# IVRL/NoiseDiff

Measured on AMD Instinct MI355X. Metric: sampled RAW patches/sec (256x256x4, 1000-step DDPM), higher is better.
Workload: dtype f32; 1 GPU; NoiseDiffNet dim=64, 256x256x4 patches, 1000-step DDPM (sigmoid2, pred_v), 16 patches per GPU; a step = one reverse-diffusion step (U-Net forward + fused posterior/noise update) over the per-GPU batch; patches/s = n_gpus*16/(1000*s_per_step); global_batch=16, launch=hipGraph replay, noise=device Philox4x32-10

## Files before the change

noisediff_amd/csrc/conv3x3_wino4.hip:

```cpp
#include <stdlib.h>
#include <type_traits>
#include "nd_common.h"

namespace {

typedef float f32x2 __attribute__((ext_vector_type(2)));
typedef unsigned u32x4_t __attribute__((ext_vector_type(4)));
typedef __attribute__((address_space(3))) void* lds_ptr;
typedef __attribute__((address_space(3))) short* lds_short_ptr;
typedef __attribute__((address_space(3))) unsigned* lds_u32_ptr;
typedef __attribute__((address_space(3))) unsigned short* lds_u16_ptr;
typedef __attribute__((address_space(3))) f32x4* lds_f32x4_ptr;

constexpr int KC4 = 16;
constexpr int NPOS = 36;
constexpr int VD_FLOATS = NPOS * 256;

constexpr int MAX_COUT = 2048;
template <int NTG, int NW = 4>
struct W4Geo {
    static constexpr int NT = 64 * NW;
    static constexpr int TGW = NTG * 4 / NW;
    static constexpr int REG_W = 16 * NTG, HALO_W = REG_W + 2;
    static constexpr int RAW_ROWP = NTG == 2 ? 40 : 24;
// ... 22 lines not shown
#ifndef W4_UR_GEN
#define W4_UR_GEN 6
#endif
#ifndef W4_UR_EPI
#define W4_UR_EPI 6
#endif
#ifndef W4_VR
#define W4_VR 3
#endif
#ifndef W4_COMMIT_AT
#define W4_COMMIT_AT 8
#endif
#ifndef W4_XF_AT
#define W4_XF_AT 10
#endif
#ifndef W4_U_AUX
#define W4_U_AUX 0
#endif
#ifndef W4_STORE_AUX
#define W4_STORE_AUX 19
#endif
#ifndef W4_STAGGER
#define W4_STAGGER 12
#endif
#ifndef W4_XF_SPLIT
#define W4_XF_SPLIT 1
#endif
#ifndef W4_UR1
#define W4_UR1 9
#endif
#ifndef W4_UR1_AFF
#define W4_UR1_AFF 6
#endif
#ifndef W4_UR1_EPI
#define W4_UR1_EPI 0
#endif
#ifndef W4_UR1_XF
#define W4_UR1_XF 6
#endif
#ifndef W4_PAIR_SKEW
#define W4_PAIR_SKEW 2
#endif
#ifndef W4_PRIO
#define W4_PRIO 0
#endif
#ifndef W4_ABLATE
#define W4_ABLATE 0
#endif

struct Wino4Args {
    nd_conv3x3 d;
    int tiles_x, tiles_y, regions_x, n_tiles, n_cg, n_c8, slots, total_wg;
    int splits, chunks_per_split;
};

#ifndef W4_NOP
#define W4_NOP ""
#endif
#define W4_MFMA_A(acc, uv, vv)  asm volatile(W4_NOP "v_mfma_f32_16x16x4_f32 %0, %2, %1, %0" : "+a"(acc) : "v"(uv), "v"(vv))
#define W4_MFMA_V(acc, uv, vv)  asm volatile(W4_NOP "v_mfma_f32_16x16x4_f32 %0, %2, %1, %0" : "+v"(acc) : "v"(uv), "v"(vv))
#define W4_MFMA_AZ(acc, uv, vv) asm volatile(W4_NOP "v_mfma_f32_16x16x4_f32 %0, %2, %1, 0" : "=&a"(acc) : "v"(uv), "v"(vv))
#define W4_MFMA_VZ(acc, uv, vv) asm volatile(W4_NOP "v_mfma_f32_16x16x4_f32 %0, %2, %1, 0" : "=&v"(acc) : "v"(uv), "v"(vv))
#define W4_MFMA_DRAIN() asm volatile("s_nop 15\n\ts_nop 15" ::: "memory")

__device__ __forceinline__ void w4_bt(const f32x2 (&d)[6], f32x2 (&t)[6]) {
    const f32x2 c4 = {4.0f, 4.0f}, cm4 = {-4.0f, -4.0f}, cm5 = {-5.0f, -5.0f}, c2 = {2.0f, 2.0f}, cm2 = {-2.0f, -2.0f};
    const f32x2 p = __builtin_elementwise_fma(cm4, d[2], d[4]), q = __builtin_elementwise_fma(cm4, d[1], d[3]);
    const f32x2 r = d[4] - d[2], s = d[3] - d[1];
    t[0] = __builtin_elementwise_fma(c4, d[0], __builtin_elementwise_fma(cm5, d[2], d[4]));
    t[1] = p + q;
    t[2] = p - q;
    t[3] = __builtin_elementwise_fma(c2, s, r);
    t[4] = __builtin_elementwise_fma(cm2, s, r);
    t[5] = __builtin_elementwise_fma(c4, d[1], __builtin_elementwise_fma(cm5, d[3], d[5]));
}

template <int HALF>
__device__ __forceinline__ void w4_bt_half(const f32x2 (&d)[6], f32x2 (&t)[3]) {
    const f32x2 c4 = {4.0f, 4.0f}, cm4 = {-4.0f, -4.0f}, cm5 = {-5.0f, -5.0f}, c2 = {2.0f, 2.0f}, cm2 = {-2.0f, -2.0f};
    if (HALF == 0) {
        const f32x2 p = __builtin_elementwise_fma(cm4, d[2], d[4]), q = __builtin_elementwise_fma(cm4, d[1], d[3]);
        t[0] = __builtin_elementwise_fma(c4, d[0], __builtin_elementwise_fma(cm5, d[2], d[4]));
        t[1] = p + q;
        t[2] = p - q;
    } else {
        const f32x2 r = d[4] - d[2], s = d[3] - d[1];
        t[0] = __builtin_elementwise_fma(c2, s, r);
        t[1] = __builtin_elementwise_fma(cm2, s, r);
        t[2] = __builtin_elementwise_fma(c4, d[1], __builtin_elementwise_fma(cm5, d[3], d[5]));
    }
}

template <int MODE, bool STREAM, bool SPLIT = false, int NTG = 2, int NW = 4>
__global__ __launch_bounds__((64 * NW), (W4Geo<NTG, NW>::WG_PER_CU)) void wino4_kernel(const Wino4Args a) {
    using Geo = W4Geo<NTG, NW>;
    constexpr int NT = Geo::NT, TGW = Geo::TGW;
    constexpr int RAW_FLOATS = Geo::RAW_FLOATS, BIAS_OFF_BYTES = Geo::BIAS_OFF_BYTES, ACC_AGPR = Geo::ACC_AGPR, REG_W = Geo::REG_W, HALO_W = Geo::HALO_W;
    constexpr bool MAP = MODE == ND_PRO_AFFINE_MAP_SILU;
    constexpr bool GEN = MODE == ND_PRO_AFFINE_GENMAP_SILU;
    constexpr bool MAPX = MAP || GEN;
    constexpr bool AFF = MODE == ND_PRO_AFFINE_SILU || MAPX;
    constexpr bool LEAKY = MODE == ND_PRO_LEAKY || MODE == ND_PRO_LEAKY_SECOND;
    constexpr int UR = TGW == 1 ? (AFF ? W4_UR1_AFF : W4_UR1) : MAP ? W4_UR_MAP : GEN ? W4_UR_GEN : AFF ? W4_UR_AFF : W4_UR, UR_EPI = TGW == 1 ? W4_UR1_EPI : W4_UR_EPI;
    static_assert(TGW == 2 || !MAPX, "the map prologues (20 more staging registers per halo item in flight) stay on the 512-register form");
    extern __shared__ __attribute__((aligned(16))) float lds_[];
    float* const Vd = lds_ + RAW_FLOATS;

    const int tid = threadIdx.x, lane = tid & 63;
    const int wave = __builtin_amdgcn_readfirstlane(tid >> 6);
    const int mtg = NW == 8 ? wave >> 2 : 0;
    const int tg = TGW == 2 ? wave >> 1 : mtg, rh = (wave >> 1) & 1, ch2 = wave & 1;
    const int tile = lane & 15, kq = lane >> 4;

    const int wgid = nd_xcd_remap(blockIdx.x, gridDim.x);
    const int t_begin = (int)((long)wgid * a.total_wg / gridDim.x), t_end = (int)((long)(wgid + 1) * a.total_wg / gridDim.x);
    if (t_begin >= t_end) return;

#ifdef W4_STAMP
    const unsigned long long stamp_c0 = __builtin_amdgcn_s_memtime(), stamp_r0 = __builtin_amdgcn_s_memrealtime();
    unsigned long long stamp_epi = 0, stamp_xf = 0, stamp_wait = 0, stamp_t = 0, stamp_drain = 0, stamp_first = 0, stamp_last = 0, stamp_second = 0, stamp_third = 0, stamp_pro = 0, stamp_top = 0, stamp_tile = 0;
#define W4_T0() (stamp_t = __builtin_amdgcn_s_memtime())
#define W4_ACC(x) (x += __builtin_amdgcn_s_memtime() - stamp_t)
#else
#define W4_T0()
#define W4_ACC(x)
#endif
#if W4_STAGGER
    if (a.total_wg >= 4 * (int)gridDim.x)
        for (int k = (int)(blockIdx.x >> 3) & 15; k > 0; --k) __builtin_amdgcn_s_sleep(W4_STAGGER);
#endif
#if W4_PAIR_SKEW
    if (NTG == 1 && 2 * blockIdx.x >= gridDim.x)
        for (int k = 0; k < W4_PAIR_SKEW; ++k) __builtin_amdgcn_s_sleep(32);
#endif
    const nd_src& s = a.d.src;
    const int H = a.d.H, W = a.d.W, Cin = a.d.cin, Cout = a.d.cout;
    const int up = s.upsample ? 1 : 0;
    const int sH = H >> up, sW = W >> up;
    const int Ctot = s.c0 + s.c1;
    const int n_chunks = SPLIT ? a.chunks_per_split : (Cin + KC4 - 1) / KC4;

    auto decode = [&](int t, int& b_, int& ty_, int& rx_, int& nt_, int& sp_) {
        int lid = t;
        nt_ = lid % a.n_tiles;  lid /= a.n_tiles;
        rx_ = lid % a.regions_x;  lid /= a.regions_x;
        ty_ = lid % a.tiles_y;
        b_ = lid / a.tiles_y;
        sp_ = 0;
        if (SPLIT) { sp_ = b_ / a.d.B;  b_ -= sp_ * a.d.B; }
    };

    constexpr int RAW_ROWP = Geo::RAW_ROWP, RAW_IT = Geo::RAW_IT;
    const long npx = (long)a.d.B * sH * sW;
    const unsigned PX_MARK = (unsigned)(npx + sW + 2);
    auto src_rsrc = [&](const float* p, long px_stride_floats) {
        return __builtin_amdgcn_make_buffer_rsrc(const_cast<float*>(p) - (long)(sW + 1) * px_stride_floats, 0,
                                                 (int)((npx + sW + 1) * px_stride_floats * 4), 0x00020000);
    };
    const __amdgpu_buffer_rsrc_t rsrc0 = src_rsrc(s.p0, s.ld0);
    const __amdgpu_buffer_rsrc_t rsrc1 = s.p1 ? src_rsrc(s.p1, s.ld1) : rsrc0;
    const __amdgpu_buffer_rsrc_t rsrcm = MAP ? src_rsrc(s.map, 2 * Ctot) : GEN ? src_rsrc(s.map, 8) : rsrc0;
    const int map_shift = s.map_blocked ? 64 : Ctot * 4;
    float* const vd_tg = Vd + tg * VD_FLOATS;
    char* const rawbuf = reinterpret_cast<char*>(lds_);
    lds_u32_ptr const ptab = (lds_u32_ptr)(Vd + NTG * VD_FLOATS) + tid;
    auto cperm = [](int c) { return ((c >> 2) & 3) | ((c & 3) << 2) | (c & 48); };
    auto swz = [](int r, int c) { return (2 * ((r >> 2) & 3)) ^ (4 * ((c >> 3) & 1)); };
    auto pixl_of = [](int t) { return GEN ? 16 * (t >> 6) + (t & 15) : t >> 2; };
    const int sq = GEN ? (tid >> 4) & 3 : tid & 3;
    lds_u32_ptr const rtab = ptab + RAW_IT * NT;
    lds_u16_ptr const dtab = (lds_u16_ptr)(ptab - tid + (Geo::RTAB ? 2 : 1) * RAW_IT * NT) + tid;
    lds_u16_ptr const ttab = dtab + RAW_IT * NT;
    float* const bias_lds = reinterpret_cast<float*>(reinterpret_cast<char*>(lds_) + BIAS_OFF_BYTES);
    auto item_rc = [&](int k, int tid_) {
        const int pix = pixl_of(tid_) + (NT / 4) * k, r = pix / HALO_W, c = pix - HALO_W * r;
        const int dy = up ? (r + 1) >> 1 : r, dx = up ? (c + 1) >> 1 : c;
        return (unsigned)(dy * sW + dx) | ((unsigned)r << 16) | ((unsigned)c << 24);
    };
#pragma unroll
    for (int k = 0; k < RAW_IT; ++k) {
        const int pix = pixl_of(tid) + (NT / 4) * k, r = pix / HALO_W, c = pix - HALO_W * r;
        dtab[k * NT] = (unsigned short)((r * RAW_ROWP + cperm(c)) * 64 + (((2 * sq) ^ swz(r, c)) * 8));
        if (Geo::RTAB) rtab[k * NT] = item_rc(k, tid);
    }
    const int t_tile = ((lane >> 1) & 7) | ((lane >> 4) & 1) << 3, t_kq = (lane & 1) | ((lane >> 5) << 1);
#pragma unroll
    for (int h = 0; h < 2; ++h)
#pragma unroll
        for (int bx = 0; bx < 6; ++bx) {
            const int r0 = 4 * (t_tile >> 2) + 4 * h, c = 16 * tg + 4 * (t_tile & 3) + bx;
            ttab[(h * 6 + bx) * NT] = (unsigned short)((4 * (t_tile >> 2) * RAW_ROWP + cperm(c)) * 64 + (((4 * ch2 + t_kq) ^ swz(r0, c)) * 8));
        }
    const unsigned t_lds = (unsigned)(ch2 * 1024 + (t_kq >> 1) * 512 + t_tile * 32 + (t_kq & 1) * 16);
    if (Geo::BIAS_LDS)
        for (int i = tid; i < a.n_tiles * 64; i += NT) bias_lds[i] = (a.d.bias && i < Cout) ? a.d.bias[i] : 0.0f;
    const __amdgpu_buffer_rsrc_t brsrc = __builtin_amdgcn_make_buffer_rsrc(const_cast<float*>(a.d.bias ? a.d.bias : a.d.weight), 0, a.d.bias ? Cout * 4 : 0, 0x00020000);
    float bias_r = 0.0f;

    const unsigned OOB = 0x7FFFFFF0u;
    int sb_ = 0;
    unsigned spx_ = 0;
    bool tab_clean = false;
    f32x4 tA4 = {1, 1, 1, 1}, tD4 = {0, 0, 0, 0};
    auto stage_tile = [&](int b_, int ty_, int rx_) {
        sb_ = b_;
        spx_ = (unsigned)((b_ * sH + ((ty_ * 16) >> up)) * sW + ((rx_ * REG_W) >> up));
        const int r_lo = ty_ == 0 ? 1 : 0, r_n = min(17, H - ty_ * 16) - r_lo;
        const int c_lo = rx_ == 0 ? 1 : 0, c_n = min(HALO_W - 1, W - rx_ * REG_W) - c_lo;
        const bool interior = r_lo == 0 && r_n == 17 && c_lo == 0 && c_n == HALO_W - 1;
        if (!(interior && tab_clean)) {
            int tid_ = tid;
            if (!Geo::RTAB) asm volatile("" : "+v"(tid_));
#pragma unroll
            for (int k = 0; k < RAW_IT; ++k) {
                const unsigned rc = Geo::RTAB ? rtab[k * NT] : item_rc(k, tid_);
                const unsigned r = (rc >> 16) & 255u, c = rc >> 24;
                const bool ok = r - (unsigned)r_lo <= (unsigned)r_n && c - (unsigned)c_lo <= (unsigned)c_n;
                ptab[k * NT] = ok ? (rc & 0xFFFFu) : PX_MARK;
            }
        }
        tab_clean = interior;
    };
    f32x4 raw[RAW_IT];
    constexpr int GEN_H = RAW_IT / 2;
    f32x4 msc[MAP ? RAW_IT : GEN ? GEN_H : 1], msh[MAP ? RAW_IT : GEN ? GEN_H : 1];
    float ev0[GEN ? RAW_IT : 1], ev1[GEN ? RAW_IT : 1];
    float gw_sc0 = 0, gw_sc1 = 0, gw_sh0 = 0, gw_sh1 = 0;
    f32x4 gb_sc = {0, 0, 0, 0}, gb_sh = {0, 0, 0, 0};
    int i_eoff = 0;
    bool i_second = false;
    __amdgpu_buffer_rsrc_t i_rs = rsrc0;
    int i_soff = 0, i_mapoff = 0;
    unsigned i_ld4 = 0, i_bias = 0;
    auto stage_issue_begin = [&](int cb_) {
        const bool sec = cb_ >= s.c0;
        i_second = sec;
        i_mapoff = (int)(cb_ * (s.map_blocked ? 8u : 4u) + spx_ * (unsigned)(2 * Ctot * 4));
        i_rs = sec ? rsrc1 : rsrc0;
        i_ld4 = (unsigned)(sec ? s.ld1 : s.ld0) * 4u;
        i_soff = (int)((sec ? cb_ - s.c0 : cb_) * 4u + spx_ * i_ld4);
        i_bias = cb_ + 4 * sq < Cin ? 16u * sq : OOB;
        if (GEN) {
            i_eoff = (int)(spx_ * 32u);
            const float* wr = s.gamma + (size_t)(cb_ + (lane & 15)) * 8 + sq;
            gw_sc0 = wr[0];  gw_sc1 = wr[4];  gw_sh0 = wr[(size_t)Ctot * 8];  gw_sh1 = wr[(size_t)Ctot * 8 + 4];
            gb_sc = nd_ld4(s.beta + cb_ + 4 * sq);  gb_sh = nd_ld4(s.beta + Ctot + cb_ + 4 * sq);
        }
        if (AFF) {
            const int c = cb_ + 4 * sq;
            const float* m = s.mad + (size_t)sb_ * 3 * Ctot + (c < Cin ? c : 0);
            const f32x4 M = nd_ld4(m), A = nd_ld4(m + Ctot), D = nd_ld4(m + 2 * Ctot);
            tA4 = A;
            tD4 = D - M * A;
        }
    };
    auto stage_issue_one = [&](int k, unsigned px, auto tile_first_c) {
#if !(W4_ABLATE & 1)
        const unsigned voff = __umul24(px, i_ld4) + i_bias;
        raw[k] = __builtin_bit_cast(f32x4, __builtin_amdgcn_raw_buffer_load_b128(i_rs, voff, i_soff, 0));
        if (GEN && decltype(tile_first_c)::value) {
            const unsigned eo = __umul24(px, 32u) + 4u * sq;
            ev0[k] = __builtin_bit_cast(float, __builtin_amdgcn_raw_buffer_load_b32(rsrcm, eo, i_eoff, 0));
            ev1[k] = __builtin_bit_cast(float, __builtin_amdgcn_raw_buffer_load_b32(rsrcm, eo, i_eoff + 16, 0));
        }
        if (MAP) {
            const unsigned mo = __umul24(px, (unsigned)(2 * Ctot * 4)) + i_bias;
            msc[k] = __builtin_bit_cast(f32x4, __builtin_amdgcn_raw_buffer_load_b128(rsrcm, mo, i_mapoff, 0));
            msh[k] = __builtin_bit_cast(f32x4, __builtin_amdgcn_raw_buffer_load_b128(rsrcm, mo, i_mapoff + map_shift, 0));
// ... 153 lines not shown
        __builtin_amdgcn_sched_barrier(0);
#pragma unroll
        for (int pp = 0; pp < 18; ++pp) {
            if (pp + W4_VR - 1 < 18) read_v(v0base, v1base, pp + W4_VR - 1);
            pre(pp);
            const f32x4 u = U[(OFF + pp) % UR];
            const f32x4 va = Vr[pp % W4_VR][0], vb = Vr[pp % W4_VR][TGW - 1];
            __builtin_amdgcn_sched_barrier(0);
            if (TGW == 2) {
                mfma(first_c, 4 * pp + 0, u.x, va.x);
                mfma(first_c, 4 * pp + 1, u.x, vb.x);
                mfma(first_c, 4 * pp + 2, u.z, va.z);
                mfma(first_c, 4 * pp + 3, u.z, vb.z);
                mfma(std::false_type{}, 4 * pp + 0, u.y, va.y);
                mfma(std::false_type{}, 4 * pp + 1, u.y, vb.y);
                mfma(std::false_type{}, 4 * pp + 2, u.w, va.w);
                mfma(std::false_type{}, 4 * pp + 3, u.w, vb.w);
            } else {
                mfma(first_c, 2 * pp + 0, u.x, va.x);
                mfma(first_c, 2 * pp + 1, u.z, va.z);
                mfma(std::false_type{}, 2 * pp + 0, u.y, va.y);
                mfma(std::false_type{}, 2 * pp + 1, u.w, va.w);
            }
            __builtin_amdgcn_sched_barrier(0);
#pragma unroll
            for (int q = (hi(pp) > DIN ? hi(pp) : DIN); q < hi(pp + 1); ++q) {
                if (q < 18) load_u(OFF + q, q, wb);
                else load_u(OFF + q, q - 18, nb);
            }
            mid(pp);
            __builtin_amdgcn_sched_barrier(0);
        }
    };

    auto read_acc2 = [&](int idx, int h) -> f32x2 {
        if (idx >= ACC_AGPR) {
            asm volatile("" : "+v"(acc[idx]));
            return h ? f32x2{acc[idx].z, acc[idx].w} : f32x2{acc[idx].x, acc[idx].y};
        }
        f32x2 r;
        if (h == 0) {
            asm volatile("v_accvgpr_read_b32 %0, %1" : "=v"(r.x) : "a"(acc[idx].x));
            asm volatile("v_accvgpr_read_b32 %0, %1" : "=v"(r.y) : "a"(acc[idx].y));
        } else {
            asm volatile("v_accvgpr_read_b32 %0, %1" : "=v"(r.x) : "a"(acc[idx].z));
            asm volatile("v_accvgpr_read_b32 %0, %1" : "=v"(r.y) : "a"(acc[idx].w));
        }
        return r;
    };

    int b, ty, rx, nt, sp;
    decode(t_begin, b, ty, rx, nt, sp);
    int b1 = b, ty1 = ty, rx1 = rx, nt1 = nt, sp1 = sp;
    stage_tile(b, ty, rx);
    stage_issue_begin(SPLIT ? sp * n_chunks * KC4 : 0);
#pragma unroll
    for (int k = 0; k < RAW_IT; ++k) stage_issue_one(k, ptab[k * NT], std::true_type{});
    {
        const int wb = wblock(SPLIT ? 2 * sp * n_chunks : 0, nt * 4 + (wave & 3));
#pragma unroll
        for (int q = 0; q < UR_EPI; ++q) load_u(q, q, wb);
    }
#pragma unroll
    for (int k = 0; k < RAW_IT; ++k) {
        if (GEN && k % GEN_H == 0) gen_maps(k);
        stage_commit_one(k, dtab[k * NT], AFF ? ptab[k * NT] : 0u);
    }
    asm volatile("s_waitcnt lgkmcnt(0)" ::: "memory");
    __builtin_amdgcn_s_barrier();
    if constexpr (TGW == 2) {
        f32x2 T[6][6];
        unsigned t_addr[12];
        xf_addr(t_addr);
#pragma unroll
        for (int ay = 0; ay < 6; ++ay) xf_read(T, t_addr, ay);
        xf_finish(T, vd_tg, [] {});
    } else xf_half(vd_tg);
    asm volatile("s_waitcnt lgkmcnt(0)" ::: "memory");
    __builtin_amdgcn_s_barrier();

#ifdef W4_STAMP
    stamp_pro = __builtin_amdgcn_s_memtime() - stamp_c0;
#endif
    for (int t = t_begin; t < t_end; ++t) {
        const bool more = t + 1 < t_end;
        W4_T0();
        if (more) {
            nt1 = nt + 1;  rx1 = rx;  ty1 = ty;  b1 = b;  sp1 = sp;
            if (nt1 == a.n_tiles) { nt1 = 0;  if (++rx1 == a.regions_x) { rx1 = 0;  if (++ty1 == a.tiles_y) { ty1 = 0;  ++b1;  if (SPLIT && b1 == a.d.B) { b1 = 0;  ++sp1; } } } }
        }
        const int ch0 = SPLIT ? sp * n_chunks : 0, ch0n = SPLIT ? sp1 * n_chunks : 0;
        const int cg = nt * 4 + (wave & 3), cg_next = (more ? nt1 : nt) * 4 + (wave & 3);

        auto chunk = [&](int ch, auto first_c, auto last_c) {
            const char* v0cur = reinterpret_cast<const char*>(Vd + mtg * VD_FLOATS) + d_lds;
            const char* v1cur = reinterpret_cast<const char*>(Vd + (NTG - 1) * VD_FLOATS) + d_lds;
            constexpr bool last = decltype(last_c)::value;
            const int c8 = 2 * (ch0 + ch);
            const int w0 = wblock(c8, cg), w1 = wblock(c8 + 1, cg), wn = last ? wblock(2 * ch0n, cg_next) : wblock(c8 + 2, cg);
#ifdef W4_STAMP
            if (decltype(first_c)::value) W4_ACC(stamp_top);
            W4_T0();
#endif
            if (last && more) stage_tile(b1, ty1, rx1);
#ifdef W4_STAMP
            if (last) W4_ACC(stamp_tile);
#endif
            using I0 = std::integral_constant<int, 0>;
            using IOFF1 = std::integral_constant<int, 18 % UR>;
            using IUR = std::integral_constant<int, UR>;
            using IEPI = std::integral_constant<int, UR_EPI>;
            using IXF = std::integral_constant<int, TGW == 1 ? (W4_UR1_XF < UR ? W4_UR1_XF : UR) : UR>;
            constexpr bool FIRST = decltype(first_c)::value;
            unsigned tab1 = 0;
            constexpr bool PRE_P = AFF && !MAPX;
            unsigned tabd[(AFF || LEAKY) ? RAW_IT : 1], tabp[PRE_P ? RAW_IT : 1];
            auto issue_pre = [&](int pp) { if (pp < RAW_IT) tab1 = ptab[pp * NT]; };
            auto issue = [&](int pp) {
                if (pp == 0) stage_issue_begin(last ? ch0n * KC4 : (ch0 + ch + 1) * KC4);
                if (pp < RAW_IT) stage_issue_one(pp, tab1, last_c);
            };
            auto commit_pre = [&](int pp) {
                if (AFF || LEAKY) {
                    if (pp == W4_COMMIT_AT) {
#pragma unroll
                        for (int k = 0; k < RAW_IT; ++k) {
                            tabd[k] = dtab[k * NT];
                            if (PRE_P) tabp[k] = ptab[k * NT];
                        }
                    }
                } else if (pp < RAW_IT) tab1 = dtab[pp * NT];
            };
            f32x2 T[TGW == 2 ? 6 : 1][6];
            unsigned t_addr[12];
            auto commit = [&](int pp) {
                if (AFF || LEAKY) {
                    if (pp == W4_COMMIT_AT) {
#pragma unroll
                        for (int k = 0; k < RAW_IT; ++k) {
                            if (GEN && k % GEN_H == 0) gen_maps(k);
                            stage_commit_one(k, tabd[(AFF || LEAKY) ? k : 0], PRE_P ? tabp[PRE_P ? k : 0] : MAPX ? ptab[k * NT] : 0u);
                        }
                    }
                } else if (pp < RAW_IT) stage_commit_one(pp, tab1, 0u);
                if constexpr (TGW == 2) {
                    if (pp == W4_XF_AT) {
                        asm volatile("s_waitcnt lgkmcnt(0)" ::: "memory");
                        __builtin_amdgcn_s_barrier();
                        xf_addr(t_addr);
                    }
                    if (pp > W4_XF_AT && pp <= W4_XF_AT + 6) xf_read(T, t_addr, pp - W4_XF_AT - 1);
                }
            };
            W4_T0();
            if (TGW == 1 && FIRST)
                bias_r = __builtin_bit_cast(float, __builtin_amdgcn_raw_buffer_load_b32(brsrc, (unsigned)(cg * 16 + (lane & 15)) * 4u, 0, 0));
            stage(first_c, I0{}, std::conditional_t<FIRST, IEPI, IXF>{}, IUR{}, v0cur, v1cur, w0, w1, issue_pre, issue);
// ... 122 lines not shown
#else
                                asm volatile("" :: "v"(v));
#endif
                            }
                        }
                    }
                };
                if (full) { if (want_stats) emit(std::true_type{}, std::true_type{}); else emit(std::true_type{}, std::false_type{}); }
                else { if (want_stats) emit(std::false_type{}, std::true_type{}); else emit(std::false_type{}, std::false_type{}); }
                if (a.d.stats) {
                    float fc = full ? 64.0f : cnt2.x + cnt2.y;
                    float S = sum2.x + sum2.y, Q = sq2.x + sq2.y;
                    fc += __shfl_xor(fc, 16);  S += __shfl_xor(S, 16);  Q += __shfl_xor(Q, 16);
                    fc += __shfl_xor(fc, 32);  S += __shfl_xor(S, 32);  Q += __shfl_xor(Q, 32);
                    const int slot = ty * a.tiles_x + tx;
                    if (kq == 0 && cok) {
                        fc = fmaxf(fc, 1.0f);
                        float* o = a.d.stats + (((size_t)b * a.slots + slot) * Cout + co) * 2;
                        *reinterpret_cast<f32x2*>(o) = f32x2{S + fc * pivot, fmaxf(Q - S * S / fc, 0.0f)};
                    }
#ifndef W4_STAMP
                    if (b == 0 && nt == 0 && (wave & 3) == 0 && lane == 0) {
                        a.d.slot_count[slot] = (float)(min(16, H - ty * 16) * min(16, W - tx * 16));
                    }
#endif
                }
            }
        }
        if (TGW == 1 && W4_PRIO) __builtin_amdgcn_s_setprio(0);
        W4_ACC(stamp_epi);
#ifdef W4_STAMP_DRAIN
        W4_T0();
        asm volatile("s_waitcnt vmcnt(0)" ::: "memory");
        W4_ACC(stamp_drain);
#endif
        b = b1; ty = ty1; rx = rx1; nt = nt1; sp = sp1;
    }
#ifdef W4_STAMP
    if (tid == 0) {
        unsigned long long* dbg = reinterpret_cast<unsigned long long*>(a.d.slot_count) + 16 * blockIdx.x;
        dbg[0] = __builtin_amdgcn_s_memtime() - stamp_c0;
        dbg[1] = __builtin_amdgcn_s_memrealtime() - stamp_r0;
        dbg[2] = (unsigned long long)(t_end - t_begin) * n_chunks;
        dbg[3] = stamp_epi;
        dbg[4] = stamp_xf;
        dbg[5] = stamp_second;
        dbg[6] = stamp_first;
        dbg[7] = stamp_last;
        dbg[8] = stamp_third;
        dbg[9] = stamp_wait;
        dbg[10] = stamp_pro;
        dbg[11] = stamp_top;
        dbg[12] = stamp_tile;
    }
#endif
}

__global__ __launch_bounds__(256) void w4_splitk_reduce_kernel(const float* __restrict__ part, const float* __restrict__ bias, float* __restrict__ out,
                                                               int splits, long npix, int cout, int ldo) {
    const int cq = cout >> 2;
    const long total = npix * cq;
    for (long i = blockIdx.x * (long)blockDim.x + threadIdx.x; i < total; i += (long)gridDim.x * blockDim.x) {
        const long n = i / cq;
        const int c = (int)(i - n * cq) * 4;
        f32x4 acc = nd_ld4(part + n * cout + c);
        for (int s = 1; s < splits; ++s) acc += nd_ld4(part + ((long)s * npix + n) * cout + c);
        if (bias) acc += nd_ld4(bias + c);
        nd_st4(out + n * ldo + c, acc);
    }
}

__global__ __launch_bounds__(256) void w4_splitk_reduce_stats_kernel(const float* __restrict__ part, const float* __restrict__ bias, float* __restrict__ out,
                                                                     float* __restrict__ stats, float* __restrict__ slot_count, int splits, int B, int H, int W,
                                                                     int cout, int ldo, int tiles_x, int tiles_y, int n_cgrp) {
    __shared__ __attribute__((aligned(16))) float red[2][256][4];
    int bid = blockIdx.x;
    const int cgrp = bid % n_cgrp;  bid /= n_cgrp;
    const int slot = bid % (tiles_x * tiles_y), b = bid / (tiles_x * tiles_y);
    const int ty = slot / tiles_x, tx = slot % tiles_x;
    const int y0 = ty * 16, x0 = tx * 16, th = min(16, H - y0), tw = min(16, W - x0), npx = th * tw;
    const long npix = (long)B * H * W;
    const int q = cgrp * 16 + (threadIdx.x & 15), rg = threadIdx.x >> 4;
    const bool act = 4 * q < cout;
    f32x4 s1 = {0, 0, 0, 0}, s2 = {0, 0, 0, 0}, pv = {0, 0, 0, 0};
    if (act) {
        const f32x4 bq = bias ? nd_ld4(bias + 4 * q) : f32x4{0, 0, 0, 0};
        {
            const long n0 = ((long)b * H + y0) * W + x0;
            pv = nd_ld4(part + n0 * cout + 4 * q);
            for (int sp = 1; sp < splits; ++sp) pv += nd_ld4(part + ((long)sp * npix + n0) * cout + 4 * q);
            pv += bq;
        }
        for (int p = rg; p < npx; p += 16) {
            const int py = p / tw, px = p - py * tw;
            const long n = ((long)b * H + y0 + py) * W + x0 + px;
            f32x4 v = nd_ld4(part + n * cout + 4 * q);
            for (int sp = 1; sp < splits; ++sp) v += nd_ld4(part + ((long)sp * npix + n) * cout + 4 * q);
            v += bq;
            nd_st4(out + n * ldo + 4 * q, v);
            const f32x4 dv = v - pv;
            s1 += dv;  s2 += dv * dv;
        }
    }
    *reinterpret_cast<f32x4*>(red[0][threadIdx.x]) = s1;
    *reinterpret_cast<f32x4*>(red[1][threadIdx.x]) = s2;
    __syncthreads();
// ... 81 lines not shown
    if (int e = nd_reserve_lds(configured, reinterpret_cast<const void*>(wino4_kernel<MODE, STREAM, false, NTG, NW>), LDS_BYTES, "nd_conv3x3_wino4")) return e;
    const long resident = (long)nd_device_cus() * W4Geo<NTG, NW>::WG_PER_CU;
    hipLaunchKernelGGL((wino4_kernel<MODE, STREAM, false, NTG, NW>), dim3((unsigned)(a.total_wg < resident ? a.total_wg : resident)), dim3(64 * NW), LDS_BYTES, st, a);
    return 0;
}

template <int MODE, int NTG = 2, int NW = 4>
int launch4(const Wino4Args& a, hipStream_t st) {
    static const long stream_min = (getenv("ND_W4_STREAM_MB") ? atol(getenv("ND_W4_STREAM_MB")) : 48) << 20;
    static const int stream_kinds = getenv("ND_W4_STREAM_KINDS") ? atoi(getenv("ND_W4_STREAM_KINDS")) : 7;
    const int kind = (MODE == ND_PRO_AFFINE_SILU || MODE == ND_PRO_AFFINE_MAP_SILU || MODE == ND_PRO_AFFINE_GENMAP_SILU) ? 2 : a.d.stats ? 1 : 4;
    const long out_bytes = (long)a.d.B * a.d.H * a.d.W * a.d.ldo * 4;
    return (out_bytes >= stream_min && (stream_kinds & kind)) ? launch4s<MODE, true, NTG, NW>(a, st) : launch4s<MODE, false, NTG, NW>(a, st);
}

}

extern "C" int64_t nd_pack_conv3x3_wino4_weight_floats(int cin, int cout) {
    return (int64_t)nd_round_up(nd_cdiv(cin, 8), 2) * nd_cdiv(nd_round_up(cout, 64), 16) * 18 * 256;
}

static int pack_wino4(const float* oihw, float* packed, int cin, int cout, int dgrad, void* stream) {
    ND_REQUIRE(oihw && packed, ND_E_BADARG, "nd_pack_conv3x3_wino4_weight: null pointer");
    ND_REQUIRE(cin > 0 && cout > 0, ND_E_BADARG, "nd_pack_conv3x3_wino4_weight: non-positive size");
    const int n_c8 = nd_round_up(nd_cdiv(cin, 8), 2), n_cg = nd_round_up(cout, 64) / 16;
    const size_t total = (size_t)n_c8 * n_cg * 64;
    const int blocks = (int)((total + 255) / 256 < 4096 ? (total + 255) / 256 : 4096);
    if (dgrad) hipLaunchKernelGGL(pack_wino4_kernel<true>, dim3(blocks), dim3(256), 0, (hipStream_t)stream, oihw, packed, cin, cout, n_c8, n_cg);
    else hipLaunchKernelGGL(pack_wino4_kernel<false>, dim3(blocks), dim3(256), 0, (hipStream_t)stream, oihw, packed, cin, cout, n_c8, n_cg);
    return nd_launch_status("nd_pack_conv3x3_wino4_weight");
}

extern "C" int nd_pack_conv3x3_wino4_weight(const float* oihw, float* packed, int cin, int cout, void* stream) {
    return pack_wino4(oihw, packed, cin, cout, 0, stream);
}

extern "C" int nd_pack_conv3x3_wino4_weight_dgrad(const float* oihw_fwd, float* packed, int cin, int cout, void* stream) {
    return pack_wino4(oihw_fwd, packed, cin, cout, 1, stream);
}

extern "C" int nd_pack_conv3x3_wino4_weights_batch(const nd_pack_item* items_dev, int n_items, void* stream) {
    ND_REQUIRE(items_dev && n_items > 0 && n_items <= 65535, ND_E_BADARG, "nd_pack_conv3x3_wino4_weights_batch: needs 1 .. 65535 items in device memory");
    hipLaunchKernelGGL(pack_wino4_batch_kernel, dim3(64, (unsigned)n_items), dim3(256), 0, (hipStream_t)stream, items_dev);
    return nd_launch_status("nd_pack_conv3x3_wino4_weights_batch");
}

extern "C" int nd_conv3x3_wino4_stat_slots(int H, int W) { return nd_cdiv(W, 16) * nd_cdiv(H, 16); }

static int w4_prepare(const nd_conv3x3* d, Wino4Args& a, int ntg = 2) {
    ND_REQUIRE(d, ND_E_BADARG, "nd_conv3x3_wino4: null descriptor");
    const nd_src& s = d->src;
    ND_REQUIRE(s.p0 && d->weight && d->out, ND_E_BADARG, "nd_conv3x3_wino4: null tensor pointer");
    ND_REQUIRE(d->B > 0 && d->H > 0 && d->W > 0 && d->cin > 0 && d->cout > 0, ND_E_BADARG, "nd_conv3x3_wino4: non-positive size");
    ND_REQUIRE(d->cin % 4 == 0 && d->cout % 4 == 0 && d->cin > KC4 && d->cout <= MAX_COUT, ND_E_SHAPE,
               "nd_conv3x3_wino4: cin=%d and cout=%d must be multiples of 4, cin > 16 (at least two K chunks), cout <= %d", d->cin, d->cout, MAX_COUT);
    ND_REQUIRE(s.c0 + s.c1 == d->cin && s.c0 % 4 == 0 && s.c1 % 4 == 0 && s.c0 > 0, ND_E_SHAPE,
               "nd_conv3x3_wino4: source channels %d+%d do not match cin=%d (multiples of 4)", s.c0, s.c1, d->cin);
    ND_REQUIRE((s.c1 == 0) == (s.p1 == nullptr), ND_E_BADARG, "nd_conv3x3_wino4: p1/c1 mismatch");
    ND_REQUIRE(s.ld0 >= s.c0 && s.ld0 % 4 == 0 && (s.c1 == 0 || (s.ld1 >= s.c1 && s.ld1 % 4 == 0)), ND_E_ALIGN,
               "nd_conv3x3_wino4: pixel strides must be >= channels and multiples of 4");
    ND_REQUIRE(nd_aligned16(s.p0) && nd_aligned16(s.p1) && nd_aligned16(d->weight) && nd_aligned16(s.mad) && nd_aligned16(d->out) &&
               nd_aligned16(d->bias), ND_E_ALIGN, "nd_conv3x3_wino4: pointers must be 16-byte aligned");
    ND_REQUIRE(d->ldo >= d->cout && d->ldo % 4 == 0, ND_E_SHAPE, "nd_conv3x3_wino4: ldo must be >= cout and a multiple of 4");
    const bool aff = s.mode == ND_PRO_AFFINE_SILU || s.mode == ND_PRO_AFFINE_MAP_SILU || s.mode == ND_PRO_AFFINE_GENMAP_SILU;
    ND_REQUIRE(s.mode == ND_PRO_NONE || aff || s.mode == ND_PRO_LEAKY || s.mode == ND_PRO_LEAKY_SECOND, ND_E_BADARG,
               "nd_conv3x3_wino4: unsupported prologue %d", s.mode);
    ND_REQUIRE(s.mode != ND_PRO_AFFINE_GENMAP_SILU || (ntg == 2 && s.map && s.gamma && s.beta && !s.upsample && !s.map_blocked && s.c1 == 0 && s.c0 % KC4 == 0 &&
                                                     nd_aligned16(s.map) && nd_aligned16(s.gamma) && nd_aligned16(s.beta)), ND_E_BADARG,
               "nd_conv3x3_wino4: the in-kernel map prologue needs silu(pos_emb) (map), mlp[1].weight (gamma) and mlp[1].bias (beta), 16-byte aligned, one source of whole "
               "16-channel chunks, no upsample addressing, the 16 x 32-region form");
    ND_REQUIRE(!aff || s.mad, ND_E_BADARG, "nd_conv3x3_wino4: affine prologue needs mad");
    ND_REQUIRE(s.mode != ND_PRO_AFFINE_MAP_SILU || (s.map && !s.upsample && nd_aligned16(s.map)), ND_E_BADARG,
               "nd_conv3x3_wino4: the map prologue needs a 16-byte aligned map and no upsample addressing");
    ND_REQUIRE(s.mode != ND_PRO_AFFINE_MAP_SILU || (long)(d->B * (long)d->H + 2) * d->W * 2 * (s.c0 + s.c1) * 4 < (1L << 30) - 65536, ND_E_SHAPE,
               "nd_conv3x3_wino4: a scale / shift map of 1 GiB or more");
    ND_REQUIRE(s.mode != ND_PRO_LEAKY_SECOND || s.p1, ND_E_BADARG, "nd_conv3x3_wino4: LEAKY_SECOND needs a second source");
    ND_REQUIRE(!s.map_blocked || (s.mode == ND_PRO_AFFINE_MAP_SILU && (s.c0 + s.c1) % 16 == 0), ND_E_BADARG,
               "nd_conv3x3_wino4: map_blocked needs the map prologue and a channel count that is a multiple of 16");
    ND_REQUIRE(!s.unshuffle, ND_E_BADARG, "nd_conv3x3_wino4: no unshuffle addressing");
    ND_REQUIRE(!s.upsample || (d->H % 2 == 0 && d->W % 2 == 0 && s.c1 == 0), ND_E_SHAPE,
               "nd_conv3x3_wino4: nearest-x2 upsample addressing needs even H, W and a single source");
    ND_REQUIRE((d->stats == nullptr) == (d->slot_count == nullptr), ND_E_BADARG, "nd_conv3x3_wino4: stats and slot_count go together");
    ND_REQUIRE(s.c1 == 0 || s.c0 % KC4 == 0, ND_E_SHAPE,
               "nd_conv3x3_wino4: first concat source has %d channels; a 16-channel K chunk must not straddle the sources", s.c0);
    ND_REQUIRE(d->W <= 2048 && d->H <= 32768, ND_E_SHAPE, "nd_conv3x3_wino4: image wider than 2048 (16-bit border table)");
    {
        const long px = (long)(d->B) * (d->H >> (s.upsample ? 1 : 0)) * (d->W >> (s.upsample ? 1 : 0));
        const long ext = px + (d->W >> (s.upsample ? 1 : 0)) + 2;
        ND_REQUIRE(ext * s.ld0 * 4 < (1L << 30) - 65536 && ext * s.ld1 * 4 < (1L << 30) - 65536 && ext < (1L << 24), ND_E_SHAPE,
                   "nd_conv3x3_wino4: a source tensor of 1 GiB or 16 M pixels or more");
    }

    ND_REQUIRE((long)d->B * d->H * d->W * d->ldo * 4 < (1L << 32) - 65536, ND_E_SHAPE, "nd_conv3x3_wino4: an output tensor of 4 GiB or more");

    a.d = *d;
    a.tiles_x = nd_cdiv(d->W, 16);
    a.tiles_y = nd_cdiv(d->H, 16);
    a.regions_x = nd_cdiv(d->W, 16 * ntg);
    a.n_tiles = nd_cdiv(d->cout, 64);
    a.n_cg = nd_round_up(d->cout, 64) / 16;
    a.n_c8 = nd_round_up(nd_cdiv(d->cin, 8), 2);
    a.slots = a.tiles_x * a.tiles_y;
    const long wg = (long)d->B * a.regions_x * a.tiles_y * a.n_tiles;
    ND_REQUIRE(wg < (1L << 31), ND_E_SHAPE, "nd_conv3x3_wino4: grid too large");
    a.total_wg = (int)wg;
    a.splits = 1;
    a.chunks_per_split = nd_cdiv(d->cin, KC4);
    return 0;
}

static int w4_splitk(const nd_conv3x3* d, float* workspace, int splits, void* stream, int ntg, const char* who) {
    Wino4Args a;
    if (int e = w4_prepare(d, a, ntg)) return e;
    ND_REQUIRE(workspace && nd_aligned16(workspace), ND_E_BADARG, "%s: the workspace must be a 16-byte aligned pointer", who);
    ND_REQUIRE(d->src.mode == ND_PRO_NONE || d->src.mode == ND_PRO_AFFINE_SILU, ND_E_BADARG,
               "%s: plain or GroupNorm-affine + SiLU sources (no map / LeakyReLU prologue)", who);
    const int n_chunks = nd_cdiv(d->cin, KC4);
    ND_REQUIRE((splits == 2 || splits == 4 || splits == 8) && d->cin % KC4 == 0 && n_chunks % splits == 0 && n_chunks / splits >= 2, ND_E_SHAPE,
               "%s: splits=%d must be 2, 4 or 8 and divide cin=%d into ranges of at least two whole 16-channel chunks", who, splits, d->cin);
    const long npix = (long)d->B * d->H * d->W;
    ND_REQUIRE((long)splits * npix * d->cout * 4 < (1L << 31), ND_E_SHAPE, "%s: partial sums of 2 GiB or more", who);
    ND_REQUIRE(d->cout % 4 == 0, ND_E_SHAPE, "%s: cout must be a multiple of 4", who);
    const float* bias = d->bias;
    float* out = d->out;
    const int ldo = d->ldo;
    a.d.out = workspace;  a.d.ldo = d->cout;  a.d.bias = nullptr;
    a.d.stats = nullptr;  a.d.slot_count = nullptr;
    a.splits = splits;
    a.chunks_per_split = n_chunks / splits;
    a.total_wg *= splits;
    hipStream_t st = (hipStream_t)stream;
    const bool aff = d->src.mode == ND_PRO_AFFINE_SILU;
    if (int rc = ntg == 1 ? (aff ? launch4_split<ND_PRO_AFFINE_SILU, 1>(a, st) : launch4_split<ND_PRO_NONE, 1>(a, st))
                          : (aff ? launch4_split<ND_PRO_AFFINE_SILU>(a, st) : launch4_split<ND_PRO_NONE>(a, st))) return rc;
    if (int e = nd_launch_status(who)) return e;
    if (d->stats) {
        const int n_cgrp = nd_cdiv(d->cout, 64);
        hipLaunchKernelGGL(w4_splitk_reduce_stats_kernel, dim3((unsigned)(d->B * a.tiles_x * a.tiles_y * n_cgrp)), dim3(256), 0, st, workspace, bias, out,
                           d->stats, d->slot_count, splits, d->B, d->H, d->W, d->cout, ldo, a.tiles_x, a.tiles_y, n_cgrp);
        return nd_launch_status(who);
    }
    const long total = npix * (d->cout / 4);
    const int blocks = (int)((total + 255) / 256 < 4096 ? (total + 255) / 256 : 4096);
    hipLaunchKernelGGL(w4_splitk_reduce_kernel, dim3(blocks), dim3(256), 0, st, workspace, bias, out, splits, npix, d->cout, ldo);
    return nd_launch_status(who);
}

extern "C" int nd_conv3x3_wino4_nhwc_f32(const nd_conv3x3* d, void* stream) {
    Wino4Args a;
    if (int e = w4_prepare(d, a)) return e;
    const nd_src& s = d->src;
    hipStream_t st = (hipStream_t)stream;
    int rc;
    switch (s.mode) {
        case ND_PRO_AFFINE_SILU: rc = launch4<ND_PRO_AFFINE_SILU>(a, st); break;
        case ND_PRO_AFFINE_MAP_SILU: rc = launch4<ND_PRO_AFFINE_MAP_SILU>(a, st); break;
        case ND_PRO_AFFINE_GENMAP_SILU: rc = launch4<ND_PRO_AFFINE_GENMAP_SILU>(a, st); break;
        case ND_PRO_LEAKY: rc = launch4<ND_PRO_LEAKY>(a, st); break;
        case ND_PRO_LEAKY_SECOND: rc = launch4<ND_PRO_LEAKY_SECOND>(a, st); break;
        default: rc = launch4<ND_PRO_NONE>(a, st); break;
// ... 52 lines not shown
```

Measured before the change: 0.9656 patches/s.

## Precompute Winograd LDS address tables at compile time and use reciprocal division

Replaces the per-workgroup computation of the staging, transform and halo address tables with constexpr tables held in device memory. Each thread loads its packed table column with vector loads and copies it to LDS. Tile-index decoding switches from integer div/mod to host-computed multiply-shift reciprocals, and the first bias element is fetched early. It also relaxes the cin > 16 requirement so a single-chunk input walks two chunks. The goal is a shorter kernel prologue, at the cost of extra global table loads, more registers and added complexity.

```diff
diff --git a/noisediff_amd/csrc/conv3x3_wino4.hip b/noisediff_amd/csrc/conv3x3_wino4.hip
--- a/noisediff_amd/csrc/conv3x3_wino4.hip
+++ b/noisediff_amd/csrc/conv3x3_wino4.hip
@@ -98,7 +98,87 @@
     nd_conv3x3 d;
     int tiles_x, tiles_y, regions_x, n_tiles, n_cg, n_c8, slots, total_wg;
     int splits, chunks_per_split;
+    unsigned rcp_m[4];
+    int rcp_s[4];
 };
+
+inline void w4_rcp(int d, unsigned& m, int& s) {
+    int l = 0;
+    while ((1L << l) < d) ++l;
+    m = (unsigned)((((unsigned long)1 << (31 + l)) + (unsigned long)d - 1) / (unsigned long)d);
+    s = 31 + l;
+}
+__device__ __forceinline__ int w4_div(int n, unsigned m, int s) { return (int)(((unsigned long long)(unsigned)n * m) >> s); }
+
+constexpr int w4_cperm(int c) { return ((c >> 2) & 3) | ((c & 3) << 2) | (c & 48); }
+constexpr int w4_swz(int r, int c) { return (2 * ((r >> 2) & 3)) ^ (4 * ((c >> 3) & 1)); }
+constexpr int w4_pixl(bool gen, int t) { return gen ? 16 * (t >> 6) + (t & 15) : t >> 2; }
+constexpr int w4_sq(bool gen, int t) { return gen ? (t >> 4) & 3 : t & 3; }
+
+struct alignas(16) W4Col { unsigned w[4]; };
+template <int NTG, int NW, bool GEN>
+struct W4Tables {
+    using Geo = W4Geo<NTG, NW>;
+    static constexpr int NT = Geo::NT, RAW_IT = Geo::RAW_IT;
+    static constexpr int D_H = 0, T_H = (RAW_IT + 1) / 2 * 2, RC_H = T_H + 12;
+    static constexpr int NV = (RC_H + RAW_IT + 7) / 8;
+    W4Col v[NV * NT];
+    constexpr unsigned half(int t, int i) const { return (v[(i >> 3) * NT + t].w[(i >> 1) & 3] >> (16 * (i & 1))) & 0xFFFFu; }
+};
+
+template <int NTG, int NW, bool GEN>
+constexpr W4Tables<NTG, NW, GEN> w4_make_tables() {
+    using Tab = W4Tables<NTG, NW, GEN>;
+    using Geo = W4Geo<NTG, NW>;
+    constexpr int NT = Geo::NT, RAW_IT = Geo::RAW_IT, HALO_W = Geo::HALO_W, RAW_ROWP = Geo::RAW_ROWP, TGW = Geo::TGW;
+    Tab T{};
+    for (int tid = 0; tid < NT; ++tid) {
+        unsigned h[Tab::NV * 8] = {};
+        const int lane = tid & 63, wave = tid >> 6, sq = w4_sq(GEN, tid);
+        for (int k = 0; k < RAW_IT; ++k) {
+            const int pix = w4_pixl(GEN, tid) + (NT / 4) * k, r = pix / HALO_W, c = pix - HALO_W * r;
+            h[Tab::D_H + k] = (unsigned short)((r * RAW_ROWP + w4_cperm(c)) * 64 + (((2 * sq) ^ w4_swz(r, c)) * 8));
+            h[Tab::RC_H + k] = (unsigned)r << 8 | (unsigned)c;
+        }
+        const int mtg = NW == 8 ? wave >> 2 : 0, tg = TGW == 2 ? wave >> 1 : mtg, ch2 = wave & 1;
+        const int t_tile = ((lane >> 1) & 7) | ((lane >> 4) & 1) << 3, t_kq = (lane & 1) | ((lane >> 5) << 1);
+        for (int hh = 0; hh < 2; ++hh)
+            for (int bx = 0; bx < 6; ++bx) {
+                const int r0 = 4 * (t_tile >> 2) + 4 * hh, c = 16 * tg + 4 * (t_tile & 3) + bx;
+                h[Tab::T_H + hh * 6 + bx] = (unsigned short)((4 * (t_tile >> 2) * RAW_ROWP + w4_cperm(c)) * 64 + (((4 * ch2 + t_kq) ^ w4_swz(r0, c)) * 8));
+            }
+        for (int j = 0; j < Tab::NV; ++j)
+            for (int i = 0; i < 4; ++i) T.v[j * NT + tid].w[i] = h[8 * j + 2 * i] | h[8 * j + 2 * i + 1] << 16;
+    }
+    return T;
+}
+
+constexpr W4Tables<2, 4, false> w4_tab2_c = w4_make_tables<2, 4, false>();
+constexpr W4Tables<2, 4, true> w4_tab2g_c = w4_make_tables<2, 4, true>();
+constexpr W4Tables<1, 4, false> w4_tab1_c = w4_make_tables<1, 4, false>();
+__device__ const W4Tables<2, 4, false> w4_tab2 = w4_tab2_c;
+__device__ const W4Tables<2, 4, true> w4_tab2g = w4_tab2g_c;
+__device__ const W4Tables<1, 4, false> w4_tab1 = w4_tab1_c;
+template <int NTG, int NW, bool GEN>
+__device__ __forceinline__ const W4Col* w4_tables() {
+    static_assert(NW == 4 && (NTG == 2 || !GEN), "no table set for this form");
+    if constexpr (NTG == 1) return w4_tab1.v; else if constexpr (GEN) return w4_tab2g.v; else return w4_tab2.v;
+}
+static_assert(W4Tables<2, 4, false>::NV == 4 && W4Tables<2, 4, false>::T_H == 10 && W4Tables<2, 4, false>::RC_H == 22, "16 x 32 form: 64 bytes per thread");
+static_assert(W4Tables<1, 4, false>::NV == 3 && W4Tables<1, 4, false>::T_H == 6 && W4Tables<1, 4, false>::RC_H == 18, "16 x 16 form: 48 bytes per thread");
+static_assert(w4_tab2_c.half(0, 0) == 0 && w4_tab2_c.half(0, 22) == 0, "thread 0, item 0: halo (0, 0)");
+static_assert(w4_tab2_c.half(0, 1) == 4320 && w4_tab2_c.half(0, 23) == (1 << 8 | 30), "thread 0, item 1: pixel 64 = halo (1, 30), record 40 + 27, slot 4");
+static_assert(w4_tab2_c.half(0, 9) == 43008 && w4_tab2_c.half(0, 31) == (16 << 8 | 32), "thread 0, item 9: pixel 576 = halo (16, 32)");
+static_assert(w4_tab2_c.half(0, 10) == 0 && w4_tab2_c.half(0, 21) == 336, "thread 0: patch columns 0 (rows 0-3) and 5 (rows 4-5: slot 2)");
+static_assert(w4_tab2_c.half(255, 0) == 4048 && w4_tab2_c.half(255, 22) == (1 << 8 | 29), "thread 255, item 0: pixel 63 = halo (1, 29), quad 3");
+static_assert(w4_tab2_c.half(255, 9) == 48016 && w4_tab2_c.half(255, 31) == (18 << 8 | 27), "thread 255, item 9: pixel 639 is beyond pixel 611: row 18");
+static_assert(w4_tab2_c.half(255, 10) == 31976 && w4_tab2_c.half(255, 21) == 33080, "thread 255: tile 15 of tile group 1, channel pair 7");
+static_assert(w4_tab2_c.half(17, 0) == 80 && w4_tab2_c.half(17, 22) == 4, "plain lane order, thread 17: pixel 4, quad 1");
+static_assert(w4_tab2g_c.half(17, 0) == 272 && w4_tab2g_c.half(17, 22) == 1, "GEN lane order, thread 17: pixel 1, quad 1");
+static_assert(w4_tab2g_c.half(255, 9) == 48016 && w4_tab2g_c.half(255, 31) == (18 << 8 | 27) && w4_tab2g_c.half(255, 21) == 33080, "GEN lane order, thread 255: as the plain order");
+static_assert(w4_tab1_c.half(0, 1) == 5280 && w4_tab1_c.half(0, 19) == (3 << 8 | 10), "16 x 16 form, thread 0, item 1: pixel 64 = halo (3, 10)");
+static_assert(w4_tab1_c.half(255, 23) == (21 << 8 | 5), "16 x 16 form, thread 255, item 5: pixel 383 is beyond pixel 323");
+static_assert(w4_tab1_c.half(255, 17) == 19768, "16 x 16 form, thread 255: patch column 5 of rows 4-5 = halo column 17");
 
 #ifndef W4_NOP
 #define W4_NOP ""
@@ -164,13 +244,20 @@
 
 #ifdef W4_STAMP
     const unsigned long long stamp_c0 = __builtin_amdgcn_s_memtime(), stamp_r0 = __builtin_amdgcn_s_memrealtime();
-    unsigned long long stamp_epi = 0, stamp_xf = 0, stamp_wait = 0, stamp_t = 0, stamp_drain = 0, stamp_first = 0, stamp_last = 0, stamp_second = 0, stamp_third = 0, stamp_pro = 0, stamp_top = 0, stamp_tile = 0;
+    unsigned long long stamp_epi = 0, stamp_xf = 0, stamp_wait = 0, stamp_t = 0, stamp_drain = 0, stamp_first = 0, stamp_last = 0, stamp_second = 0, stamp_third = 0, stamp_pro = 0, stamp_top = 0, stamp_tile = 0, stamp_p1 = 0, stamp_p2 = 0, stamp_p3 = 0;
 #define W4_T0() (stamp_t = __builtin_amdgcn_s_memtime())
 #define W4_ACC(x) (x += __builtin_amdgcn_s_memtime() - stamp_t)
 #else
 #define W4_T0()
 #define W4_ACC(x)
 #endif
+    using Tab = W4Tables<NTG, NW, GEN>;
+    u32x4_t tcol[Tab::NV];
+#pragma unroll
+    for (int j = 0; j < Tab::NV; ++j) tcol[j] = *reinterpret_cast<const u32x4_t*>(w4_tables<NTG, NW, GEN>() + j * NT + tid);
+    auto thalf = [&](int i) -> unsigned { const unsigned w = tcol[i >> 3][(i >> 1) & 3];  return (i & 1) ? w >> 16 : w & 0xFFFFu; };
+    float bias_early = 0.0f;
+    if (Geo::BIAS_LDS) bias_early = (a.d.bias && tid < a.d.cout) ? a.d.bias[tid] : 0.0f;
 #if W4_STAGGER
     if (a.total_wg >= 4 * (int)gridDim.x)
         for (int k = (int)(blockIdx.x >> 3) & 15; k > 0; --k) __builtin_amdgcn_s_sleep(W4_STAGGER);
@@ -184,16 +271,15 @@
     const int up = s.upsample ? 1 : 0;
     const int sH = H >> up, sW = W >> up;
     const int Ctot = s.c0 + s.c1;
-    const int n_chunks = SPLIT ? a.chunks_per_split : (Cin + KC4 - 1) / KC4;
+    const int n_chunks = SPLIT ? a.chunks_per_split : max(2, (Cin + KC4 - 1) / KC4);
 
     auto decode = [&](int t, int& b_, int& ty_, int& rx_, int& nt_, int& sp_) {
-        int lid = t;
-        nt_ = lid % a.n_tiles;  lid /= a.n_tiles;
-        rx_ = lid % a.regions_x;  lid /= a.regions_x;
-        ty_ = lid % a.tiles_y;
-        b_ = lid / a.tiles_y;
+        int lid = t, q;
+        q = w4_div(lid, a.rcp_m[0], a.rcp_s[0]);  nt_ = lid - q * a.n_tiles;  lid = q;
+        q = w4_div(lid, a.rcp_m[1], a.rcp_s[1]);  rx_ = lid - q * a.regions_x;  lid = q;
+        b_ = w4_div(lid, a.rcp_m[2], a.rcp_s[2]);  ty_ = lid - b_ * a.tiles_y;
         sp_ = 0;
-        if (SPLIT) { sp_ = b_ / a.d.B;  b_ -= sp_ * a.d.B; }
+        if (SPLIT) { sp_ = w4_div(b_, a.rcp_m[3], a.rcp_s[3]);  b_ -= sp_ * a.d.B; }
     };
 
     constexpr int RAW_ROWP = Geo::RAW_ROWP, RAW_IT = Geo::RAW_IT;
@@ -210,10 +296,8 @@
     float* const vd_tg = Vd + tg * VD_FLOATS;
     char* const rawbuf = reinterpret_cast<char*>(lds_);
     lds_u32_ptr const ptab = (lds_u32_ptr)(Vd + NTG * VD_FLOATS) + tid;
-    auto cperm = [](int c) { return ((c >> 2) & 3) | ((c & 3) << 2) | (c & 48); };
-    auto swz = [](int r, int c) { return (2 * ((r >> 2) & 3)) ^ (4 * ((c >> 3) & 1)); };
-    auto pixl_of = [](int t) { return GEN ? 16 * (t >> 6) + (t & 15) : t >> 2; };
-    const int sq = GEN ? (tid >> 4) & 3 : tid & 3;
+    auto pixl_of = [](int t) { return w4_pixl(GEN, t); };
+    const int sq = w4_sq(GEN, tid);
     lds_u32_ptr const rtab = ptab + RAW_IT * NT;
     lds_u16_ptr const dtab = (lds_u16_ptr)(ptab - tid + (Geo::RTAB ? 2 : 1) * RAW_IT * NT) + tid;
     lds_u16_ptr const ttab = dtab + RAW_IT * NT;
@@ -223,23 +307,27 @@
         const int dy = up ? (r + 1) >> 1 : r, dx = up ? (c + 1) >> 1 : c;
         return (unsigned)(dy * sW + dx) | ((unsigned)r << 16) | ((unsigned)c << 24);
     };
-#pragma unroll
-    for (int k = 0; k < RAW_IT; ++k) {
-        const int pix = pixl_of(tid) + (NT / 4) * k, r = pix / HALO_W, c = pix - HALO_W * r;
-        dtab[k * NT] = (unsigned short)((r * RAW_ROWP + cperm(c)) * 64 + (((2 * sq) ^ swz(r, c)) * 8));
-        if (Geo::RTAB) rtab[k * NT] = item_rc(k, tid);
-    }
+    auto item_rc_tab = [&](int k) {
+        const unsigned rc = thalf(Tab::RC_H + k), r = rc >> 8, c = rc & 255u;
+        return (((r + (unsigned)up) >> up) * (unsigned)sW + ((c + (unsigned)up) >> up)) | (r << 16) | (c << 24);
+    };
+    auto tables_to_lds = [&] {
+#pragma unroll
+        for (int k = 0; k < RAW_IT; ++k) {
+            dtab[k * NT] = (unsigned short)thalf(Tab::D_H + k);
+            if (Geo::RTAB) rtab[k * NT] = item_rc_tab(k);
+        }
+#pragma unroll
+        for (int i = 0; i < 12; ++i) ttab[i * NT] = (unsigned short)thalf(Tab::T_H + i);
+    };
     const int t_tile = ((lane >> 1) & 7) | ((lane >> 4) & 1) << 3, t_kq = (lane & 1) | ((lane >> 5) << 1);
-#pragma unroll
-    for (int h = 0; h < 2; ++h)
-#pragma unroll
-        for (int bx = 0; bx < 6; ++bx) {
-            const int r0 = 4 * (t_tile >> 2) + 4 * h, c = 16 * tg + 4 * (t_tile & 3) + bx;
-            ttab[(h * 6 + bx) * NT] = (unsigned short)((4 * (t_tile >> 2) * RAW_ROWP + cperm(c)) * 64 + (((4 * ch2 + t_kq) ^ swz(r0, c)) * 8));
-        }
     const unsigned t_lds = (unsigned)(ch2 * 1024 + (t_kq >> 1) * 512 + t_tile * 32 + (t_kq & 1) * 16);
-    if (Geo::BIAS_LDS)
-        for (int i = tid; i < a.n_tiles * 64; i += NT) bias_lds[i] = (a.d.bias && i < Cout) ? a.d.bias[i] : 0.0f;
+    auto bias_to_lds = [&] {
+        if (Geo::BIAS_LDS) {
+            if (tid < a.n_tiles * 64) bias_lds[tid] = bias_early;
+            for (int i = tid + NT; i < a.n_tiles * 64; i += NT) bias_lds[i] = (a.d.bias && i < Cout) ? a.d.bias[i] : 0.0f;
+        }
+    };
     const __amdgpu_buffer_rsrc_t brsrc = __builtin_amdgcn_make_buffer_rsrc(const_cast<float*>(a.d.bias ? a.d.bias : a.d.weight), 0, a.d.bias ? Cout * 4 : 0, 0x00020000);
     float bias_r = 0.0f;
 
@@ -248,7 +336,7 @@
     unsigned spx_ = 0;
     bool tab_clean = false;
     f32x4 tA4 = {1, 1, 1, 1}, tD4 = {0, 0, 0, 0};
-    auto stage_tile = [&](int b_, int ty_, int rx_) {
+    auto stage_tile = [&](int b_, int ty_, int rx_, auto prologue_c) {
         sb_ = b_;
         spx_ = (unsigned)((b_ * sH + ((ty_ * 16) >> up)) * sW + ((rx_ * REG_W) >> up));
         const int r_lo = ty_ == 0 ? 1 : 0, r_n = min(17, H - ty_ * 16) - r_lo;
@@ -259,7 +347,7 @@
             if (!Geo::RTAB) asm volatile("" : "+v"(tid_));
 #pragma unroll
             for (int k = 0; k < RAW_IT; ++k) {
-                const unsigned rc = Geo::RTAB ? rtab[k * NT] : item_rc(k, tid_);
+                const unsigned rc = Geo::RTAB ? rtab[k * NT] : decltype(prologue_c)::value ? item_rc_tab(k) : item_rc(k, tid_);
                 const unsigned r = (rc >> 16) & 255u, c = rc >> 24;
                 const bool ok = r - (unsigned)r_lo <= (unsigned)r_n && c - (unsigned)c_lo <= (unsigned)c_n;
                 ptab[k * NT] = ok ? (rc & 0xFFFFu) : PX_MARK;
@@ -519,7 +607,12 @@
     int b, ty, rx, nt, sp;
     decode(t_begin, b, ty, rx, nt, sp);
     int b1 = b, ty1 = ty, rx1 = rx, nt1 = nt, sp1 = sp;
-    stage_tile(b, ty, rx);
+    tables_to_lds();
+    bias_to_lds();
+#ifdef W4_STAMP
+    stamp_p1 = __builtin_amdgcn_s_memtime() - stamp_c0;
+#endif
+    stage_tile(b, ty, rx, std::true_type{});
     stage_issue_begin(SPLIT ? sp * n_chunks * KC4 : 0);
 #pragma unroll
     for (int k = 0; k < RAW_IT; ++k) stage_issue_one(k, ptab[k * NT], std::true_type{});
@@ -528,6 +621,9 @@
 #pragma unroll
         for (int q = 0; q < UR_EPI; ++q) load_u(q, q, wb);
     }
+#ifdef W4_STAMP
+    stamp_p2 = __builtin_amdgcn_s_memtime() - stamp_c0;
+#endif
 #pragma unroll
     for (int k = 0; k < RAW_IT; ++k) {
         if (GEN && k % GEN_H == 0) gen_maps(k);
@@ -535,6 +631,9 @@
     }
     asm volatile("s_waitcnt lgkmcnt(0)" ::: "memory");
     __builtin_amdgcn_s_barrier();
+#ifdef W4_STAMP
+    stamp_p3 = __builtin_amdgcn_s_memtime() - stamp_c0;
+#endif
     if constexpr (TGW == 2) {
         f32x2 T[6][6];
         unsigned t_addr[12];
@@ -569,7 +668,7 @@
             if (decltype(first_c)::value) W4_ACC(stamp_top);
             W4_T0();
 #endif
-            if (last && more) stage_tile(b1, ty1, rx1);
+            if (last && more) stage_tile(b1, ty1, rx1, std::false_type{});
 #ifdef W4_STAMP
             if (last) W4_ACC(stamp_tile);
 #endif
@@ -798,6 +897,9 @@
         dbg[10] = stamp_pro;
         dbg[11] = stamp_top;
         dbg[12] = stamp_tile;
+        dbg[13] = stamp_p1;
+        dbg[14] = stamp_p2;
+        dbg[15] = stamp_p3;
     }
 #endif
 }
@@ -985,8 +1087,9 @@
     const nd_src& s = d->src;
     ND_REQUIRE(s.p0 && d->weight && d->out, ND_E_BADARG, "nd_conv3x3_wino4: null tensor pointer");
     ND_REQUIRE(d->B > 0 && d->H > 0 && d->W > 0 && d->cin > 0 && d->cout > 0, ND_E_BADARG, "nd_conv3x3_wino4: non-positive size");
-    ND_REQUIRE(d->cin % 4 == 0 && d->cout % 4 == 0 && d->cin > KC4 && d->cout <= MAX_COUT, ND_E_SHAPE,
-               "nd_conv3x3_wino4: cin=%d and cout=%d must be multiples of 4, cin > 16 (at least two K chunks), cout <= %d", d->cin, d->cout, MAX_COUT);
+    ND_REQUIRE(d->cin % 4 == 0 && d->cout % 4 == 0 && d->cin >= KC4 && d->cout <= MAX_COUT, ND_E_SHAPE,
+               "nd_conv3x3_wino4: cin=%d and cout=%d must be multiples of 4, cin >= 16 (one K chunk; the kernel walks two, so cin > 16 is where it pays), cout <= %d",
+               d->cin, d->cout, MAX_COUT);
     ND_REQUIRE(s.c0 + s.c1 == d->cin && s.c0 % 4 == 0 && s.c1 % 4 == 0 && s.c0 > 0, ND_E_SHAPE,
                "nd_conv3x3_wino4: source channels %d+%d do not match cin=%d (multiples of 4)", s.c0, s.c1, d->cin);
     ND_REQUIRE((s.c1 == 0) == (s.p1 == nullptr), ND_E_BADARG, "nd_conv3x3_wino4: p1/c1 mismatch");
@@ -998,10 +1101,10 @@
     const bool aff = s.mode == ND_PRO_AFFINE_SILU || s.mode == ND_PRO_AFFINE_MAP_SILU || s.mode == ND_PRO_AFFINE_GENMAP_SILU;
     ND_REQUIRE(s.mode == ND_PRO_NONE || aff || s.mode == ND_PRO_LEAKY || s.mode == ND_PRO_LEAKY_SECOND, ND_E_BADARG,
                "nd_conv3x3_wino4: unsupported prologue %d", s.mode);
-    ND_REQUIRE(s.mode != ND_PRO_AFFINE_GENMAP_SILU || (ntg == 2 && s.map && s.gamma && s.beta && !s.upsample && !s.map_blocked && s.c1 == 0 && s.c0 % KC4 == 0 &&
+    ND_REQUIRE(s.mode != ND_PRO_AFFINE_GENMAP_SILU || (ntg == 2 && s.map && s.gamma && s.beta && !s.upsample && !s.map_blocked && s.c1 == 0 && s.c0 % KC4 == 0 && s.c0 > KC4 &&
                                                      nd_aligned16(s.map) && nd_aligned16(s.gamma) && nd_aligned16(s.beta)), ND_E_BADARG,
                "nd_conv3x3_wino4: the in-kernel map prologue needs silu(pos_emb) (map), mlp[1].weight (gamma) and mlp[1].bias (beta), 16-byte aligned, one source of whole "
-               "16-channel chunks, no upsample addressing, the 16 x 32-region form");
+               "16-channel chunks (two at least), no upsample addressing, the 16 x 32-region form");
     ND_REQUIRE(!aff || s.mad, ND_E_BADARG, "nd_conv3x3_wino4: affine prologue needs mad");
     ND_REQUIRE(s.mode != ND_PRO_AFFINE_MAP_SILU || (s.map && !s.upsample && nd_aligned16(s.map)), ND_E_BADARG,
                "nd_conv3x3_wino4: the map prologue needs a 16-byte aligned map and no upsample addressing");
@@ -1039,6 +1142,8 @@
     a.total_wg = (int)wg;
     a.splits = 1;
     a.chunks_per_split = nd_cdiv(d->cin, KC4);
+    const int divisors[4] = {a.n_tiles, a.regions_x, a.tiles_y, d->B};
+    for (int i = 0; i < 4; ++i) w4_rcp(divisors[i], a.rcp_m[i], a.rcp_s[i]);
     return 0;
 }
 
```

New measurement: 0.9665 patches/s, median of 3. Within noise of the previous version (+0.1%).
